# ai-decentralized/BloomBee

Measured on AMD Instinct MI355X. Metric: decode tokens/sec, llama-3-8b greedy, pipeline over RCCL/xGMI, higher is better.
Workload: dtype bfloat16; 1 GPU; model=llama-3-8b, global_batch=32, seq_len=2048, parallelism=pp1, micro_batches=1

## Files before the change

bloombee_amd/ops/hip/elementwise.hip:

```cpp

#include "common.h"


template <int BLOCK, int ITERS>
__global__ __launch_bounds__(BLOCK) void rmsnorm_kernel(
    const unsigned short* __restrict__ x, const unsigned short* __restrict__ res,
    const unsigned short* __restrict__ w, unsigned short* __restrict__ out_h,
    unsigned short* __restrict__ out_y, int H, float eps) {
  const long row = blockIdx.x;
  const unsigned short* xr = x + row * (long)H;
  const unsigned short* rr = res ? res + row * (long)H : nullptr;

  float v[ITERS][8];
  float ssq = 0.f;
#pragma unroll
  for (int it = 0; it < ITERS; ++it) {
    int d = (it * BLOCK + threadIdx.x) * 8;
    if (d < H) {
      load_bf16x8(xr + d, v[it]);
      if (rr) {
        float r[8];
        load_bf16x8(rr + d, r);
#pragma unroll
        for (int j = 0; j < 8; ++j) v[it][j] = bf2f(f2bf(v[it][j] + r[j]));
// ... 138 lines not shown
    for (int j = 0; j < 8; ++j) {
      float t = tanhf(0.7978845608028654f * (v[j] + 0.044715f * v[j] * v[j] * v[j]));
      o[j] = 0.5f * v[j] * (1.f + t);
    }
    store_bf16x8(out + idx * 8, o);
  }
  for (long i = nvec * 8 + blockIdx.x * (long)blockDim.x + threadIdx.x; i < n;
       i += (long)gridDim.x * blockDim.x) {
    const float v = bf2f(x[i]);
    const float t = tanhf(0.7978845608028654f * (v + 0.044715f * v * v * v));
    out[i] = f2bf(0.5f * v * (1.f + t));
  }
}

__global__ void add_kernel(const unsigned short* __restrict__ a,
                           const unsigned short* __restrict__ b,
                           unsigned short* __restrict__ out, long n) {
  const long nvec = n / 8;
  for (long idx = blockIdx.x * (long)blockDim.x + threadIdx.x; idx < nvec;
       idx += (long)gridDim.x * blockDim.x) {
    float va[8], vb[8], o[8];
    load_bf16x8(a + idx * 8, va);
    load_bf16x8(b + idx * 8, vb);
#pragma unroll
    for (int j = 0; j < 8; ++j) o[j] = va[j] + vb[j];
    store_bf16x8(out + idx * 8, o);
  }
  for (long i = nvec * 8 + blockIdx.x * (long)blockDim.x + threadIdx.x; i < n;
       i += (long)gridDim.x * blockDim.x)
    out[i] = f2bf(bf2f(a[i]) + bf2f(b[i]));
}


template <bool PART>
__global__ void rope_kv_write_kernel(
    unsigned short* __restrict__ qkv, const float* __restrict__ part,
    const unsigned short* __restrict__ bias, int ksplit,
    const float* __restrict__ cos_t,
    const float* __restrict__ sin_t, const int* __restrict__ pos,
    unsigned short* __restrict__ k_pages, unsigned short* __restrict__ v_pages,
    const int* __restrict__ page_table, const int* __restrict__ start_pos,
    int B, int Hq, int Hkv, int T, int D, int P, int maxp, int max_pos,
    int* __restrict__ ctx_out = nullptr) {
  constexpr int V = PART ? 4 : 1;
  const int bt = blockIdx.x;
  const int b = bt / T, t = bt % T;
  const int h = blockIdx.y;
  if (ctx_out && h == 0 && t == 0 && threadIdx.x == 0)
    ctx_out[b] = start_pos[b] + T;
  const int X = Hq + 2 * Hkv;
  const long hoff = (((long)b * T + t) * X + h) * D;
  unsigned short* base = qkv + hoff;
  auto load = [&](int i, float* x) {
    if constexpr (PART) {
      const long total = (long)B * T * X * D;
      f32x4 v = {0.f, 0.f, 0.f, 0.f};
      for (int s = 0; s < ksplit; ++s) {
        const f32x4 p =
            *reinterpret_cast<const f32x4*>(part + s * total + hoff + i);
#pragma unroll
        for (int e = 0; e < 4; ++e) v[e] += p[e];
      }
#pragma unroll
      for (int e = 0; e < 4; ++e) {
        if (bias) v[e] += bf2f(bias[h * D + i + e]);
        x[e] = bf2f(f2bf(v[e]));
      }
    } else {
      x[0] = bf2f(base[i]);
    }
  };

  const int abspos = start_pos[b] + t;
  if (h >= Hq + Hkv) {
    const int hv = h - Hq - Hkv;
    const int page = page_table[b * maxp + abspos / P];
    const int slot = abspos % P;
    unsigned short* dst = v_pages + ((long)page * Hkv + hv) * D * P + slot;
    for (int i = threadIdx.x * V; i < D; i += blockDim.x * V) {
      if constexpr (PART) {
        float x[V];
        load(i, x);
#pragma unroll
        for (int e = 0; e < V; ++e) dst[(long)(i + e) * P] = f2bf(x[e]);
      } else {
        dst[(long)i * P] = base[i];
      }
    }
    return;
  }
  const int p = min(max(pos ? pos[b * T + t] : abspos, 0), max_pos - 1);
  const float* c = cos_t + (long)p * (D / 2);
  const float* s = sin_t + (long)p * (D / 2);
  unsigned short* dst = base;
  if (h >= Hq) {
    const int hk = h - Hq;
    const int page = page_table[b * maxp + abspos / P];
    dst = k_pages + (((long)page * Hkv + hk) * P + (abspos % P)) * D;
  }
  for (int i = threadIdx.x * V; i < D / 2; i += blockDim.x * V) {
    float xa[V], xb[V];
    load(i, xa);
    load(i + D / 2, xb);
    unsigned short oa[V], ob[V];
#pragma unroll
    for (int e = 0; e < V; ++e) {
#pragma clang fp contract(off)
      float x1 = xa[e], x2 = xb[e];
      float cc = c[i + e], ss = s[i + e];
      oa[e] = f2bf(x1 * cc - x2 * ss);
      ob[e] = f2bf(x2 * cc + x1 * ss);
    }
    if constexpr (PART) {
      *reinterpret_cast<short4v*>(dst + i) =
          (short4v){(short)oa[0], (short)oa[1], (short)oa[2], (short)oa[3]};
      *reinterpret_cast<short4v*>(dst + i + D / 2) =
          (short4v){(short)ob[0], (short)ob[1], (short)ob[2], (short)ob[3]};
    } else {
      dst[i] = oa[0];
      dst[i + D / 2] = ob[0];
    }
  }
}
```

bloombee_amd/ops/hip/ext.hip:

```cpp

#include <torch/extension.h>
#include <c10/hip/HIPStream.h>
#include <hip/hip_runtime.h>
#include <cstdlib>

#include "common.h"

#include "elementwise.hip"
#include "kvcache.hip"
#include "attn_decode.hip"
#include "attn_decode_mfma.hip"
#include "attn_sparse.hip"
#include "attn_prefill.hip"
#include "attn_train.hip"
#include "gemm_skinny.hip"
#include "moe_gemm.hip"
#include "w4_gemm.hip"
#include "moe_gemm_w4.hip"
#include "mfma_selftest.hip"
#include "quant4.hip"
#include "wire.h"

typedef __attribute__((ext_vector_type(8))) short short8_h;

// ... 105 lines not shown

static SplitK split_k_chunks(int K, int unit, int ksplit) {
  const int nch = K / unit;
  TORCH_CHECK(nch >= 1 && ksplit >= 1, "split-K needs K >= ", unit);
  const int per = (nch + ksplit - 1) / ksplit;
  return {(nch + per - 1) / per, per * unit};
}

struct SkinnyPlan {
  int ksplit, kchunk;
  bool v2;
};

static SkinnyPlan skinny_plan(long N, long K, long ksplit_req) {
  TORCH_CHECK(N >= 64 && K >= 32 && K % 32 == 0 && N % 64 == 0,
              "K%32, N%64 required");
  int ksplit = (int)ksplit_req;
  if (ksplit <= 0) {
    static const int ks_big = [] {
      const char* e = std::getenv("BBAMD_GEMM_KSPLIT_BIG");
      return e ? std::atoi(e) : 1;
    }();
    if (N / 64 >= 256) ksplit = ks_big;
    else ksplit = (int)std::min<long>(K / 512,
                                      std::max<long>(1, std::min<long>(8, 1024 / (N / 64))));
    ksplit = std::max(1, ksplit);
  }
  if (K % 256 != 0)
    return {ksplit, (int)((K / 32 + ksplit - 1) / ksplit) * 32, false};
  const SplitK s = split_k_chunks((int)K, 256, ksplit);
  return {s.ksplit, s.kchunk, true};
}

struct W4Plan {
  bool gemv;
  int ksplit, kchunk;
};

static W4Plan w4_plan(long M, long N, long K, long ksplit_req) {
  TORCH_CHECK(N >= 64 && K >= 128 && K % 128 == 0 && N % 64 == 0,
              "K%128, N%64 required");
  if (M == 1 && K % 2048 == 0 && K / 2048 <= 7) return {true, 1, (int)K};
  int ksplit = (int)ksplit_req;
  if (ksplit <= 0) {
    ksplit = (int)std::max<long>(1, std::min<long>(K / 512, 1792 / (N / 64)));
  }
  const SplitK s = split_k_chunks((int)K, 128, ksplit);
  return {false, s.ksplit, s.kchunk};
}

static SplitK moe_w4_plan(long E, long N, long K, long S, long ksplit_req) {
  TORCH_CHECK(N >= 64 && K >= 128 && K % 128 == 0 && N % 64 == 0,
              "K%128, N%64 required");
  int ksplit = (int)ksplit_req;
  if (ksplit <= 0) {
    const long blocks = (N / 64) * std::max<long>(1, std::min<long>(E, S));
    ksplit = (int)std::max<long>(1, std::min<long>(K / 512, 1792 / blocks));
  }
  return split_k_chunks((int)K, 128, ksplit);
}

std::tuple<long, long, bool> gemm_skinny_plan(long N, long K, long ksplit_req) {
  const SkinnyPlan p = skinny_plan(N, K, ksplit_req);
  return {p.ksplit, p.kchunk, p.v2};
}

std::tuple<bool, long, long> gemm_w4_plan(long M, long N, long K, long ksplit_req) {
  const W4Plan p = w4_plan(M, N, K, ksplit_req);
  return {p.gemv, p.ksplit, p.kchunk};
}

std::tuple<long, long> moe_gemm_w4_plan(long E, long N, long K, long S,
                                        long ksplit_req) {
  const SplitK p = moe_w4_plan(E, N, K, S, ksplit_req);
  return {p.ksplit, p.kchunk};
}

struct Slabs {
  torch::Tensor t;
  float* p = nullptr;
};

static Slabs alloc_slabs(const Operands& ops, const torch::Tensor& like,
                         int ksplit, long rows, long N) {
  Slabs s;
  if (ksplit > 1) {
    s.t = torch::empty({(long)ksplit, rows, N}, like.options().dtype(at::kFloat));
    s.p = ops.ptr<F32>(s.t, "part");
  }
  return s;
}

static dim3 moe_grid(int N, long E, long mchunks, int ksplit) {
  TORCH_CHECK(mchunks >= 1 && E * mchunks <= 65535,
              "E * mchunks exceeds the grid limit");
  return dim3(N / 64, (unsigned)(E * mchunks), ksplit);
}
// ... 566 lines not shown
  auto* dvp = ops.ptr<Bf16>(dv, "dv");
  float* deltap = ops.ptr<F32>(delta, "delta");
  const int ntile = t.ntile;
  const int G = (int)(Hq / Hkv);
  dispatch_head_dim<128, 64>((int)D, "attn_train", [&](auto d) {
    constexpr int DD = decltype(d)::value;
    attn_train_dq_kernel<DD><<<(unsigned)(B * Hq * ntile), 512, 0, cur_stream()>>>(
        doutp, t.q, t.k, t.v, outp, lsep, alibi_ptr, dqp, deltap, (int)Hq, G,
        (int)T, ntile, (int)window, (float)scale,
        dout.stride(0), dout.stride(1), dout.stride(2),
        q.stride(0), q.stride(1), q.stride(2), k.stride(0), k.stride(1),
        k.stride(2), v.stride(0), v.stride(1), v.stride(2));
    attn_train_dkdv_kernel<DD><<<(unsigned)(B * Hkv * ntile), 512, 0, cur_stream()>>>(
        doutp, t.q, t.k, t.v, lsep, deltap, alibi_ptr, dkp, dvp,
        (int)Hq, G, (int)T, ntile, (int)window, (float)scale,
        dout.stride(0), dout.stride(1), dout.stride(2),
        q.stride(0), q.stride(1), q.stride(2), k.stride(0), k.stride(1),
        k.stride(2), v.stride(0), v.stride(1), v.stride(2));
  });
  return {dq, dk, dv};
}

static void rope_kv_write_launch(
    const Operands& ops, torch::Tensor& qkv, const float* partp, int nslab,
    const unsigned short* biasp, int* ctxp, int B, int T, int Hq, int Hkv,
    const torch::Tensor& cos_t, const torch::Tensor& sin_t,
    const c10::optional<torch::Tensor>& pos, const PagedKV& kv,
    const torch::Tensor& start_pos, long start_numel) {
  auto* qkvp = ops.ptr<Bf16>(qkv, "qkv");
  const float* cp = ops.ptr<F32>(cos_t, "cos_t");
  const float* sp = ops.ptr<F32>(sin_t, "sin_t");
  const int* posp = ops.ptr<I32>(pos, "pos", true, partp ? (long)B * T : -1);
  const int* spp = ops.ptr<I32>(start_pos, "start_pos", true, start_numel);
  dim3 grid(B * T, Hq + 2 * Hkv);
  if (partp)
    rope_kv_write_kernel<true><<<grid, 64, 0, cur_stream()>>>(
        qkvp, partp, biasp, nslab, cp, sp, posp, kv.k, kv.v, kv.pt, spp, B, Hq,
        Hkv, T, kv.D, kv.P, kv.maxp, (int)cos_t.size(0), ctxp);
  else
    rope_kv_write_kernel<false><<<grid, 64, 0, cur_stream()>>>(
        qkvp, nullptr, nullptr, 0, cp, sp, posp, kv.k, kv.v, kv.pt, spp, B, Hq,
        Hkv, T, kv.D, kv.P, kv.maxp, (int)cos_t.size(0));
}

void rope_kv_write_(torch::Tensor qkv, long Hq_, long Hkv_, torch::Tensor cos_t,
                    torch::Tensor sin_t, c10::optional<torch::Tensor> pos,
                    torch::Tensor k_pages, torch::Tensor v_pages,
                    torch::Tensor page_table, torch::Tensor start_pos) {
  Operands ops(qkv, "qkv");
  const PagedKV kv = paged_kv(ops, k_pages, v_pages, page_table);
  const int Hq = (int)Hq_, Hkv = (int)Hkv_;
  const int B = qkv.size(0), T = qkv.size(1);
  TORCH_CHECK(qkv.size(2) == (long)(Hq + 2 * Hkv) * kv.D, "bad fused qkv shape");
  rope_kv_write_launch(ops, qkv, nullptr, 0, nullptr, nullptr, B, T, Hq, Hkv,
                       cos_t, sin_t, pos, kv, start_pos, -1);
}

std::vector<torch::Tensor> rope_kv_write_part(torch::Tensor part,
                                 c10::optional<torch::Tensor> bias, long B_,
                                 long T_, long Hq_, long Hkv_,
                                 torch::Tensor cos_t, torch::Tensor sin_t,
                                 c10::optional<torch::Tensor> pos,
                                 torch::Tensor k_pages, torch::Tensor v_pages,
                                 torch::Tensor page_table,
                                 torch::Tensor start_pos) {
  Operands ops(part, "part");
  const float* partp = ops.ptr<F32>(part, "part");
  const PagedKV kv = paged_kv(ops, k_pages, v_pages, page_table);
  const int Hq = (int)Hq_, Hkv = (int)Hkv_, B = (int)B_, T = (int)T_;
  const int D = kv.D;
  const long X = Hq + 2 * Hkv;
  TORCH_CHECK(part.dim() == 3 && part.size(1) == (long)B * T &&
              part.size(2) == X * D,
              "part must be f32 (ksplit, B*T, (Hq+2Hkv)*D)");
  TORCH_CHECK(D % 8 == 0, "rope_kv_write_part needs head_dim % 8 == 0");
// ... 122 lines not shown
  dim3 grid(N / 64, ksplit);
  dispatch_mtile(M, [&](auto mt) {
    gemm_skinny_w4_kernel<decltype(mt)::value><<<grid, 256, 0, cur_stream()>>>(
        ap, qp, scp, zp, ksplit == 1 ? rp : nullptr, ksplit == 1 ? bp : nullptr,
        cp, part.p, M, N, K, plan.kchunk, ksplit);
  });
  if (ksplit > 1) {
    const long total = (long)M * N;
    const int cgrid = (int)std::min<long>((total + 255) / 256, 2048);
    gemm_skinny_combine_kernel<<<cgrid, 256, 0, cur_stream()>>>(
        part.p, rp, bp, cp, M, N, ksplit);
  }
  return C;
}


static const float* ss_in_operand(const Operands& ops,
                                  const c10::optional<torch::Tensor>& ss_in,
                                  int* nstripes) {
  *nstripes = 0;
  if (!ss_in.has_value()) return nullptr;
  TORCH_CHECK(ss_in->numel() % 32 == 0, "ss_in must be f32 (nstripes,32)");
  *nstripes = (int)(ss_in->numel() / 32);
  return ops.ptr<F32>(*ss_in, "ss_in");
}

torch::Tensor gemm_skinny(torch::Tensor A, torch::Tensor W,
                          c10::optional<torch::Tensor> residual,
                          c10::optional<torch::Tensor> bias, long ksplit_req,
                          c10::optional<torch::Tensor> norm_w, double eps,
                          c10::optional<torch::Tensor> ss_in,
                          c10::optional<torch::Tensor> ss_out,
                          long norm_mode_req, bool defer_combine,
                          c10::optional<torch::Tensor> cnt) {
  Operands ops(A, "A");
  const auto* ap = ops.ptr<Bf16>(A, "A");
  const auto* wp = ops.ptr<Bf16>(W, "W");
  const int K = A.size(-1);
  const int M = A.numel() / K;
  const int N = W.size(0);
  TORCH_CHECK(M <= 32, "gemm_skinny is for M <= 32, got ", M);
  TORCH_CHECK(W.size(1) == K, "A/W K mismatch");
  TORCH_CHECK(K % 32 == 0 && N % 64 == 0, "K%32, N%64 required");
  int norm_mode = (int)norm_mode_req;
  const auto* nwp = ops.ptr<Bf16>(norm_w, "norm_w", true, K);
  if (nwp && norm_mode == 0) norm_mode = 1;
  TORCH_CHECK(norm_mode != 1 || nwp, "norm_mode 1 needs norm_w");
  if (norm_mode)
    TORCH_CHECK(K % 256 == 0, "fused rmsnorm needs the v2 (K%256) kernel");
  TORCH_CHECK(!ss_in.has_value() || norm_mode != 0,
              "ss_in only meaningful with a norm mode");
  int nstripes = 0;
  const float* ssinp = ss_in_operand(ops, ss_in, &nstripes);
  float* ssoutp = ops.ptr<F32>(ss_out, "ss_out", true, (long)(N / 64) * 32);
  const auto* rp = ops.ptr<Bf16>(residual, "residual", true, (long)M * N);
  const auto* bp = ops.ptr<Bf16>(bias, "bias", true, N);
  int* cntp = ops.ptr<I32>(cnt, "cnt");
  auto sizes = A.sizes().vec();
  sizes.back() = N;
  auto C = torch::empty(sizes, A.options());
  auto* cp = ops.ptr<Bf16>(C, "C");
  const SkinnyPlan plan = skinny_plan(N, K, ksplit_req);
  const int ksplit = plan.ksplit, kchunk = plan.kchunk;
  const Slabs part = alloc_slabs(ops, A, ksplit, M, N);
  if (cnt.has_value() && ksplit > 1 && plan.v2) {
    TORCH_CHECK(!defer_combine, "cnt and defer_combine exclude each other");
    TORCH_CHECK(cnt->numel() >= N / 64, "cnt must be int32 of >= N/64 entries");
    dispatch_mtile(M, [&](auto mt) {
      gemm_skinny_v2_kernel<decltype(mt)::value, 2>
          <<<dim3((N / 64) * ksplit), 256, 0, cur_stream()>>>(
              ap, wp, rp, bp, cp, part.p, M, N, K, kchunk, ksplit, nwp,
              (float)eps, norm_mode, ssinp, nstripes, ssoutp, cntp);
    });
    return C;
  }
  dim3 grid(N / 64, ksplit);
  dispatch_mtile(M, [&](auto mt) {
    if (plan.v2)
      gemm_skinny_v2_kernel<decltype(mt)::value><<<grid, 256, 0, cur_stream()>>>(
          ap, wp, ksplit == 1 ? rp : nullptr, ksplit == 1 ? bp : nullptr, cp,
          part.p, M, N, K, kchunk, ksplit, nwp, (float)eps, norm_mode, ssinp,
          nstripes, ksplit == 1 ? ssoutp : nullptr);
    else {
      TORCH_CHECK(!norm_mode && (!ssoutp || ksplit > 1),
                  "fused norm / ss_out need the v2 (K%256) kernel");
      gemm_skinny_kernel<decltype(mt)::value><<<grid, 256, 0, cur_stream()>>>(
          ap, wp, ksplit == 1 ? rp : nullptr, ksplit == 1 ? bp : nullptr, cp,
          part.p, M, N, K, ksplit);
    }
  });
  if (ksplit > 1 && defer_combine) {
    TORCH_CHECK(!rp && !ssoutp, "defer_combine takes no residual / ss_out");
    return part.t;
  }
  if (ksplit > 1) {
    if (ssoutp || (N % 64 == 0 && N / 64 >= 64)) {
      dim3 cg(N / 64, (M + 15) / 16);
      gemm_skinny_combine_ss_kernel<<<cg, 256, 0, cur_stream()>>>(
          part.p, rp, bp, cp, ssoutp, M, N, ksplit);
    } else {
      const long total = (long)M * N;
      const int cgrid = (int)std::min<long>((total + 255) / 256, 2048);
      gemm_skinny_combine_kernel<<<cgrid, 256, 0, cur_stream()>>>(
          part.p, rp, bp, cp, M, N, ksplit);
    }
  }
  return C;
}

torch::Tensor gemm_skinny_swiglu(torch::Tensor A, torch::Tensor W, double eps,
                                 c10::optional<torch::Tensor> ss_in,
                                 long norm_mode_req) {
  Operands ops(A, "A");
  const auto* ap = ops.ptr<Bf16>(A, "A");
  const auto* wp = ops.ptr<Bf16>(W, "W");
  const int K = A.size(-1);
  const int M = A.numel() / K;
  const int N = W.size(0);
  const int I = N / 2;
  const int norm_mode = (int)norm_mode_req;
  TORCH_CHECK(M >= 1 && M <= 32, "gemm_skinny_swiglu is for 1 <= M <= 32, got ", M);
  TORCH_CHECK(W.dim() == 2 && W.size(1) == K, "A/W K mismatch");
  TORCH_CHECK(N % 2 == 0 && I % 32 == 0 && K % 256 == 0,
              "gemm_skinny_swiglu needs I % 32 == 0 and K % 256 == 0");
  TORCH_CHECK(norm_mode == 0 || norm_mode == 2, "norm_mode must be 0 or 2");
  TORCH_CHECK(!ss_in.has_value() || norm_mode == 2,
              "ss_in only meaningful with norm_mode 2");
  int nstripes = 0;
  const float* ssinp = ss_in_operand(ops, ss_in, &nstripes);
  auto sizes = A.sizes().vec();
  sizes.back() = I;
  auto C = torch::empty(sizes, A.options());
  auto* cp = ops.ptr<Bf16>(C, "C");
  dispatch_mtile(M, [&](auto mt) {
    gemm_skinny_v2_kernel<decltype(mt)::value, 1>
        <<<dim3(I / 32), 256, 0, cur_stream()>>>(
            ap, wp, nullptr, nullptr, cp, nullptr, M, N, K, K, 1, nullptr,
            (float)eps, norm_mode, ssinp, nstripes, nullptr, nullptr);
  });
  return C;
}


std::vector<torch::Tensor> quant4_pack(torch::Tensor x) {
  Operands ops(x, "x");
  const auto* xp = ops.ptr<Bf16>(x, "x");
  const long ncols = x.size(-1);
  TORCH_CHECK(ncols % 64 == 0, "quant4 needs cols % 64 == 0");
  const long nrows = x.numel() / ncols;
  auto packed = torch::empty({nrows, ncols / 2}, x.options().dtype(at::kByte));
  auto scale = torch::empty({nrows, ncols / 64}, x.options().dtype(at::kHalf));
  auto zero = torch::empty_like(scale);
  const long ngroups = nrows * (ncols / 64);
  const int wpb = 4;
  quant4_pack_kernel<64><<<(ngroups + wpb - 1) / wpb, wpb * 64, 0, cur_stream()>>>(
      xp, ops.ptr<U8>(packed, "packed"), ops.ptr<F16>(scale, "scale"),
      ops.ptr<F16>(zero, "zero"), nrows, ncols);
  return {packed, scale, zero};
}

torch::Tensor quant4_unpack(torch::Tensor packed, torch::Tensor scale,
                            torch::Tensor zero) {
  Operands ops(packed, "packed");
  auto* qp = ops.ptr<U8>(packed, "packed");
  TORCH_CHECK(packed.dim() == 2, "packed must be (rows, cols/2)");
  const long nrows = packed.size(0), ncols = packed.size(1) * 2;
  TORCH_CHECK(ncols % 64 == 0, "quant4 needs cols % 64 == 0");
  auto* scp = ops.ptr<F16>(scale, "scale", true, nrows * (ncols / 64));
  auto* zp = ops.ptr<F16>(zero, "zero", true, nrows * (ncols / 64));
  auto out = torch::empty({nrows, ncols}, packed.options().dtype(at::kBFloat16));
  const long total = nrows * ncols;
// ... 32 lines not shown
  mfma_selftest_kernel<<<1, 64, 0, cur_stream()>>>(ap, bp, ops.ptr<F32>(C, "C"));
  return C;
}

PYBIND11_MODULE(TORCH_EXTENSION_NAME, m) {
  m.def("rms_norm", &rms_norm);
  m.def("rms_norm_residual", &rms_norm_residual);
  m.def("layer_norm", &layer_norm);
  m.def("rope_apply_", &rope_apply_);
  m.def("swiglu", &swiglu);
  m.def("gelu_tanh", &gelu_tanh);
  m.def("add_bf16", &add_bf16);
  m.def("kv_write", &kv_write);
  m.def("kv_gather", &kv_gather);
  m.def("wire_deflate", &wire_deflate);
  m.def("wire_inflate", &wire_inflate);
  m.def("wire_deflate_mt", &wire_deflate_mt);
  m.def("wire_inflate_mt", &wire_inflate_mt);
  m.def("attn_decode", &attn_decode);
  m.def("attn_decode_qkv", &attn_decode_qkv);
  m.def("attn_decode_mixed", &attn_decode_mixed);
  m.def("attn_decode_sparse", &attn_decode_sparse);
  m.def("attn_decode_sparse_qkv", &attn_decode_sparse_qkv);
  m.def("attn_prefill_qkv", &attn_prefill_qkv);
  m.def("rope_kv_write_", &rope_kv_write_);
  m.def("attn_prefill", &attn_prefill);
  m.def("attn_train_fwd", &attn_train_fwd);
  m.def("attn_train_bwd", &attn_train_bwd);
  m.def("gemm_skinny", &gemm_skinny, py::arg("A"), py::arg("W"),
        py::arg("residual") = c10::nullopt, py::arg("bias") = c10::nullopt,
        py::arg("ksplit") = 0, py::arg("norm_w") = c10::nullopt,
        py::arg("eps") = 0.0, py::arg("ss_in") = c10::nullopt,
        py::arg("ss_out") = c10::nullopt, py::arg("norm_mode") = 0,
        py::arg("defer_combine") = false, py::arg("cnt") = c10::nullopt);
  m.def("gemm_skinny_swiglu", &gemm_skinny_swiglu, py::arg("A"), py::arg("W"),
        py::arg("eps") = 0.0, py::arg("ss_in") = c10::nullopt,
        py::arg("norm_mode") = 0);
  m.def("gemm_skinny_plan", &gemm_skinny_plan);
  m.def("rope_kv_write_part", &rope_kv_write_part);
  m.def("moe_gemm", &moe_gemm);
  m.def("gemm_w4", &gemm_w4);
  m.def("gemm_w4_plan", &gemm_w4_plan);
  m.def("moe_gemm_w4", &moe_gemm_w4);
  m.def("moe_gemm_w4_plan", &moe_gemm_w4_plan);
  m.def("quant4_pack", &quant4_pack);
  m.def("quant4_unpack", &quant4_unpack);
  m.def("mfma_selftest", &mfma_selftest);
  m.def("kv_stream_probe", &kv_stream_probe);
}
```

bloombee_amd/ops/hip/gemm_skinny.hip:

```cpp

#include "common.h"

template <int MT>
__global__ __launch_bounds__(256) void gemm_skinny_kernel(
    const unsigned short* __restrict__ A,
    const unsigned short* __restrict__ W,
    const unsigned short* __restrict__ R,
    const unsigned short* __restrict__ bias,
    unsigned short* __restrict__ C,
    float* __restrict__ Cpart,
    int M, int N, int K, int ksplit) {
  const int wave = threadIdx.x / WAVE;
  const int lane = threadIdx.x & (WAVE - 1);
  const int li = lane & 15;
  const int hi = lane >> 4;
  const int n0 = blockIdx.x * 64 + wave * 16;
  if (n0 >= N) return;
  const int split = blockIdx.y;
  const int kchunk = ((K / 32 + ksplit - 1) / ksplit) * 32;
  const int k0 = split * kchunk;
  const int k1 = min(K, k0 + kchunk);

  const unsigned short* wrow = W + (long)(n0 + li) * K;
  int arow[MT];
// ... 58 lines not shown

DEVINL void gemm_skinny_combine_lane(
    const float* Cpart, const unsigned short* __restrict__ R,
    const unsigned short* __restrict__ bias, unsigned short* __restrict__ C,
    float* __restrict__ ssout, int M, int N, int ksplit, int stripe, int m,
    int lane) {
  const int n0 = stripe * 64;
  const int c4 = (lane & 15) * 4;
  const long total = (long)M * N;
  const long i = (long)m * N + n0 + c4;
  f32x4 v = {0.f, 0.f, 0.f, 0.f};
  for (int s = 0; s < ksplit; ++s) {
    const f32x4 p = *reinterpret_cast<const f32x4*>(Cpart + s * total + i);
#pragma unroll
    for (int e = 0; e < 4; ++e) v[e] += p[e];
  }
#pragma unroll
  for (int e = 0; e < 4; ++e) {
    if (bias) v[e] += bf2f(bias[n0 + c4 + e]);
    if (R) v[e] += bf2f(R[i + e]);
  }
  short4v o4;
#pragma unroll
  for (int e = 0; e < 4; ++e) o4[e] = (short)f2bf(v[e]);
  *reinterpret_cast<short4v*>(C + i) = o4;
  if (ssout) {
    float vs = v[0] * v[0] + v[1] * v[1] + v[2] * v[2] + v[3] * v[3];
#pragma unroll
    for (int msk = 1; msk < 16; msk <<= 1) vs += __shfl_xor(vs, msk);
    if ((lane & 15) == 0) ssout[(long)stripe * 32 + m] = vs;
  }
}

template <int MT, int EPI = 0>
__global__ __launch_bounds__(256) void gemm_skinny_v2_kernel(
    const unsigned short* __restrict__ A,
    const unsigned short* __restrict__ W,
    const unsigned short* __restrict__ R,
    const unsigned short* __restrict__ bias,
    unsigned short* __restrict__ C,
    float* __restrict__ Cpart,
    int M, int N, int K, int kchunk, int ksplit,
    const unsigned short* __restrict__ nw,
    float eps, int norm_mode,
    const float* __restrict__ ssin,
    int nstripes,
    float* __restrict__ ssout,
    int* cnt = nullptr) {
  constexpr int U = 4;
  constexpr int KSTEP = 256;
  constexpr int RSTRIDE = KSTEP + 8;
  __shared__ __attribute__((aligned(16))) unsigned short atile[32 * RSTRIDE];
  __shared__ float ssp[256];
  __shared__ float invr[32];

  const int wave = threadIdx.x / WAVE;
  const int lane = threadIdx.x & (WAVE - 1);
  const int li = lane & 15;
  const int hi = lane >> 4;
  int tile = blockIdx.x;
  {
    const int nwg = gridDim.x;
    const int xcd = tile % 8, orig8 = tile / 8;
    const int q = nwg / 8, r = nwg % 8;
    if (nwg >= 8)
      tile = (xcd < r ? xcd * (q + 1) : r * (q + 1) + (xcd - r) * q) + orig8;
  }
  int split = blockIdx.y;
  if constexpr (EPI == 2) {
    split = tile % ksplit;
    tile /= ksplit;
  }
  const int n0 = tile * 64 + wave * 16;
  const int k0 = split * kchunk;
  const int k1 = min(K, k0 + kchunk);

  const unsigned short* wrow = W + (long)(n0 + li) * K;
  if constexpr (EPI == 1)
    wrow = W + ((long)(li < 8 ? 0 : N / 2 - 8) + tile * 32 + wave * 8 + li) * K;

  f32x4 acc[MT];
#pragma unroll
  for (int t = 0; t < MT; ++t) acc[t] = (f32x4){0.f, 0.f, 0.f, 0.f};

  short8 aregs[(32 * KSTEP) / (256 * 8)];
  short8 nregs[(32 * KSTEP) / (256 * 8)];
  auto load_a = [&](int ks) {
#pragma unroll
    for (int j = 0; j < 4; ++j) {
      const int flat = threadIdx.x + j * 256;
      const int row = min(flat / 32, M - 1);
      const int off = (flat % 32) * 8;
      aregs[j] = *reinterpret_cast<const short8*>(A + (long)row * K + ks + off);
      if (norm_mode == 1)
        nregs[j] = *reinterpret_cast<const short8*>(nw + ks + off);
    }
  };
  auto store_a = [&]() {
#pragma unroll
    for (int j = 0; j < 4; ++j) {
      const int flat = threadIdx.x + j * 256;
      short8 v = aregs[j];
      if (norm_mode == 1) {
        const float ir = invr[flat / 32 >= M ? M - 1 : flat / 32];
#pragma unroll
        for (int e = 0; e < 8; ++e)
          v[e] = (short)f2bf(bf2f((unsigned short)v[e]) * ir *
                             bf2f((unsigned short)nregs[j][e]));
      }
      *reinterpret_cast<short8*>(atile + (flat / 32) * RSTRIDE + (flat % 32) * 8) =
          v;
    }
  };

  bf16x8 bB0[U], bB1[U];
  auto issue0 = [&](int k) {
#pragma unroll
    for (int u = 0; u < U; ++u)
      bB0[u] = as_bf16x8(
          *reinterpret_cast<const short8*>(wrow + k + u * 32 + hi * 8));
  };
  auto issue1 = [&](int k) {
#pragma unroll
    for (int u = 0; u < U; ++u)
      bB1[u] = as_bf16x8(
          *reinterpret_cast<const short8*>(wrow + k + u * 32 + hi * 8));
  };
  auto mfma_set = [&](bf16x8* bB, int half) {
#pragma unroll
    for (int u = 0; u < U; ++u)
#pragma unroll
      for (int t = 0; t < MT; ++t) {
        bf16x8 afrag = as_bf16x8(*reinterpret_cast<const short8*>(
            atile + (t * 16 + li) * RSTRIDE + half * 128 + u * 32 + hi * 8));
        acc[t] = __builtin_amdgcn_mfma_f32_16x16x32_bf16(afrag, bB[u], acc[t],
                                                         0, 0, 0);
      }
  };

  auto reduce_invr = [&]() {
    if (ssin) {
      const int row = threadIdx.x & 31, grp = threadIdx.x >> 5;
      float s0 = 0.f, s1 = 0.f, s2 = 0.f, s3 = 0.f;
      int s = grp;
// ... 9 lines not shown
      if (threadIdx.x < 32) {
        float t = 0.f;
#pragma unroll
        for (int g = 0; g < 8; ++g) t += ssp[g * 32 + threadIdx.x];
        invr[threadIdx.x] = rsqrtf(t / K + eps);
      }
      __syncthreads();
    } else {
      const int row = threadIdx.x >> 3, sub = threadIdx.x & 7;
      float ss = 0.f;
      if (row < M) {
        const unsigned short* p = A + (long)row * K + sub * (K / 8);
        for (int x = 0; x < K / 8; x += 8) {
          short8 v = *reinterpret_cast<const short8*>(p + x);
#pragma unroll
          for (int e = 0; e < 8; ++e) {
            const float f = bf2f((unsigned short)v[e]);
            ss += f * f;
          }
        }
      }
      ssp[threadIdx.x] = ss;
      __syncthreads();
      if (sub == 0 && row < M) {
        float t = 0.f;
#pragma unroll
        for (int e = 0; e < 8; ++e) t += ssp[(row << 3) + e];
        invr[row] = rsqrtf(t / K + eps);
      }
      __syncthreads();
    }
  };

  if (norm_mode == 1) {
    issue0(k0);
    reduce_invr();
    load_a(k0);
    store_a();
    __syncthreads();
  } else {
    load_a(k0);
    issue0(k0);
    store_a();
    __syncthreads();
  }
  for (int k = k0; k < k1; k += KSTEP) {
    if (k + KSTEP < k1) load_a(k + KSTEP);
    issue1(k + 128);
    mfma_set(bB0, 0);
    if (k + KSTEP < k1) issue0(k + KSTEP);
    mfma_set(bB1, 1);
    if (k + KSTEP < k1) {
      __syncthreads();
      store_a();
      __syncthreads();
    }
  }

  if (norm_mode == 2) reduce_invr();

  if constexpr (EPI == 1) {
    unsigned short* otile = atile;
    __syncthreads();
#pragma unroll
    for (int t = 0; t < MT; ++t)
#pragma unroll
      for (int reg = 0; reg < 4; ++reg) {
        const int m = t * 16 + hi * 4 + reg;
        float v = acc[t][reg];
        if (norm_mode == 2) v *= invr[m];
        const float g = bf2f(f2bf(v));
        const float u = __shfl_xor(g, 8);
        const float sg = g / (1.f + fast_expf(-g));
        if (li < 8) otile[m * 32 + wave * 8 + li] = f2bf(sg * u);
      }
    __syncthreads();
    if (threadIdx.x < 128) {
      const int m = threadIdx.x >> 2, c8 = (threadIdx.x & 3) * 8;
      if (m < M)
        *reinterpret_cast<short8*>(C + (long)m * (N / 2) + tile * 32 + c8) =
            *reinterpret_cast<const short8*>(otile + m * 32 + c8);
    }
    return;
  }

  if constexpr (EPI == 2) {
    constexpr int TS = 68;
    float* ftile = reinterpret_cast<float*>(atile);
    __syncthreads();
// ... 69 lines not shown
          if (m < M) {
            float v = acc[t][reg];
            if (norm_mode == 2) v *= invr[m];
            if (bias) v += bf2f(bias[n0 + li]);
            if (R) v += bf2f(R[(long)m * N + n0 + li]);
            C[(long)m * N + n0 + li] = f2bf(v);
            vs = v * v;
          }
#pragma unroll
          for (int msk = 1; msk < 16; msk <<= 1) vs += __shfl_xor(vs, msk);
          if (li == 0) ssp[wave * 32 + m] = vs;
        }
      __syncthreads();
      if (threadIdx.x < 32)
        ssout[(long)tile * 32 + threadIdx.x] =
            ssp[threadIdx.x] + ssp[32 + threadIdx.x] +
            ssp[64 + threadIdx.x] + ssp[96 + threadIdx.x];
    }
  } else {
    float* dst = Cpart + (long)split * M * N;
#pragma unroll
    for (int t = 0; t < MT; ++t)
#pragma unroll
      for (int reg = 0; reg < 4; ++reg) {
        const int m = t * 16 + hi * 4 + reg;
        if (m >= M) continue;
        float v = acc[t][reg];
        if (norm_mode == 2) v *= invr[m];
        dst[(long)m * N + n0 + li] = v;
      }
  }
}

__global__ __launch_bounds__(256) void gemm_skinny_combine_ss_kernel(
    const float* __restrict__ Cpart, const unsigned short* __restrict__ R,
    const unsigned short* __restrict__ bias, unsigned short* __restrict__ C,
    float* __restrict__ ssout, int M, int N, int ksplit) {
  const int lane = threadIdx.x & (WAVE - 1);
  const int m = blockIdx.y * 16 + (threadIdx.x >> 6) * 4 + (lane >> 4);
  if (m >= M) return;
  gemm_skinny_combine_lane(Cpart, R, bias, C, ssout, M, N, ksplit, blockIdx.x,
                           m, lane);
}

__global__ void gemm_skinny_combine_kernel(
    const float* __restrict__ Cpart, const unsigned short* __restrict__ R,
    const unsigned short* __restrict__ bias, unsigned short* __restrict__ C,
    int M, int N, int ksplit) {
  const long total = (long)M * N;
  for (long i = blockIdx.x * (long)blockDim.x + threadIdx.x; i < total;
       i += (long)gridDim.x * blockDim.x) {
    float v = 0.f;
    for (int s = 0; s < ksplit; ++s) v += Cpart[(long)s * total + i];
    if (bias) v += bf2f(bias[i % N]);
    if (R) v += bf2f(R[i]);
    C[i] = f2bf(v);
  }
}
```

Measured before the change: 5417 tokens/s.

## Add configurable W-ring prefetch depth to skinny GEMM and vectorize split-K rope write

```diff
diff --git a/bloombee_amd/ops/hip/elementwise.hip b/bloombee_amd/ops/hip/elementwise.hip
--- a/bloombee_amd/ops/hip/elementwise.hip
+++ b/bloombee_amd/ops/hip/elementwise.hip
@@ -194,44 +194,18 @@
 }
 
 
-template <bool PART>
 __global__ void rope_kv_write_kernel(
-    unsigned short* __restrict__ qkv, const float* __restrict__ part,
-    const unsigned short* __restrict__ bias, int ksplit,
-    const float* __restrict__ cos_t,
+    unsigned short* __restrict__ qkv, const float* __restrict__ cos_t,
     const float* __restrict__ sin_t, const int* __restrict__ pos,
     unsigned short* __restrict__ k_pages, unsigned short* __restrict__ v_pages,
     const int* __restrict__ page_table, const int* __restrict__ start_pos,
-    int B, int Hq, int Hkv, int T, int D, int P, int maxp, int max_pos,
-    int* __restrict__ ctx_out = nullptr) {
-  constexpr int V = PART ? 4 : 1;
+    int B, int Hq, int Hkv, int T, int D, int P, int maxp, int max_pos) {
   const int bt = blockIdx.x;
   const int b = bt / T, t = bt % T;
   const int h = blockIdx.y;
-  if (ctx_out && h == 0 && t == 0 && threadIdx.x == 0)
-    ctx_out[b] = start_pos[b] + T;
   const int X = Hq + 2 * Hkv;
   const long hoff = (((long)b * T + t) * X + h) * D;
   unsigned short* base = qkv + hoff;
-  auto load = [&](int i, float* x) {
-    if constexpr (PART) {
-      const long total = (long)B * T * X * D;
-      f32x4 v = {0.f, 0.f, 0.f, 0.f};
-      for (int s = 0; s < ksplit; ++s) {
-        const f32x4 p =
-            *reinterpret_cast<const f32x4*>(part + s * total + hoff + i);
-#pragma unroll
-        for (int e = 0; e < 4; ++e) v[e] += p[e];
-      }
-#pragma unroll
-      for (int e = 0; e < 4; ++e) {
-        if (bias) v[e] += bf2f(bias[h * D + i + e]);
-        x[e] = bf2f(f2bf(v[e]));
-      }
-    } else {
-      x[0] = bf2f(base[i]);
-    }
-  };
 
   const int abspos = start_pos[b] + t;
   if (h >= Hq + Hkv) {
@@ -239,16 +213,7 @@
     const int page = page_table[b * maxp + abspos / P];
     const int slot = abspos % P;
     unsigned short* dst = v_pages + ((long)page * Hkv + hv) * D * P + slot;
-    for (int i = threadIdx.x * V; i < D; i += blockDim.x * V) {
-      if constexpr (PART) {
-        float x[V];
-        load(i, x);
-#pragma unroll
-        for (int e = 0; e < V; ++e) dst[(long)(i + e) * P] = f2bf(x[e]);
-      } else {
-        dst[(long)i * P] = base[i];
-      }
-    }
+    for (int i = threadIdx.x; i < D; i += blockDim.x) dst[(long)i * P] = base[i];
     return;
   }
   const int p = min(max(pos ? pos[b * T + t] : abspos, 0), max_pos - 1);
@@ -260,27 +225,103 @@
     const int page = page_table[b * maxp + abspos / P];
     dst = k_pages + (((long)page * Hkv + hk) * P + (abspos % P)) * D;
   }
-  for (int i = threadIdx.x * V; i < D / 2; i += blockDim.x * V) {
-    float xa[V], xb[V];
-    load(i, xa);
-    load(i + D / 2, xb);
-    unsigned short oa[V], ob[V];
-#pragma unroll
-    for (int e = 0; e < V; ++e) {
+  for (int i = threadIdx.x; i < D / 2; i += blockDim.x) {
 #pragma clang fp contract(off)
-      float x1 = xa[e], x2 = xb[e];
-      float cc = c[i + e], ss = s[i + e];
-      oa[e] = f2bf(x1 * cc - x2 * ss);
-      ob[e] = f2bf(x2 * cc + x1 * ss);
-    }
-    if constexpr (PART) {
-      *reinterpret_cast<short4v*>(dst + i) =
-          (short4v){(short)oa[0], (short)oa[1], (short)oa[2], (short)oa[3]};
-      *reinterpret_cast<short4v*>(dst + i + D / 2) =
-          (short4v){(short)ob[0], (short)ob[1], (short)ob[2], (short)ob[3]};
-    } else {
-      dst[i] = oa[0];
-      dst[i + D / 2] = ob[0];
-    }
-  }
-}
+    float x1 = bf2f(base[i]), x2 = bf2f(base[i + D / 2]);
+    float cc = c[i], ss = s[i];
+    dst[i] = f2bf(x1 * cc - x2 * ss);
+    dst[i + D / 2] = f2bf(x2 * cc + x1 * ss);
+  }
+}
+
+__global__ __launch_bounds__(256) void rope_kv_write_part_kernel(
+    unsigned short* __restrict__ qkv, const float* __restrict__ part,
+    const unsigned short* __restrict__ bias, int ksplit,
+    const float* __restrict__ cos_t, const float* __restrict__ sin_t,
+    const int* __restrict__ pos, unsigned short* __restrict__ k_pages,
+    unsigned short* __restrict__ v_pages, const int* __restrict__ page_table,
+    const int* __restrict__ start_pos, int B, int Hq, int Hkv, int T, int D,
+    int P, int maxp, int max_pos, int* __restrict__ ctx_out) {
+  constexpr int NS = 8;
+  const int bt = blockIdx.x;
+  const int b = bt / T, t = bt % T;
+  if (blockIdx.y == 0 && t == 0 && threadIdx.x == 0)
+    ctx_out[b] = start_pos[b] + T;
+  const int X = Hq + 2 * Hkv;
+  const int item = blockIdx.y * blockDim.x + threadIdx.x;
+  if (item >= X * (D / 8)) return;
+  const int h = item / (D / 8);
+  const int i = (item % (D / 8)) * 4;
+  const long total = (long)B * T * X * D;
+  const long hoff = ((long)bt * X + h) * D;
+
+  f32x4 pa[NS], pb[NS];
+#pragma unroll
+  for (int s = 0; s < NS; ++s) {
+    const float* src = part + min(s, ksplit - 1) * total + hoff + i;
+    pa[s] = *reinterpret_cast<const f32x4*>(src);
+    pb[s] = *reinterpret_cast<const f32x4*>(src + D / 2);
+  }
+  f32x4 va = {0.f, 0.f, 0.f, 0.f}, vb = {0.f, 0.f, 0.f, 0.f};
+#pragma unroll
+  for (int s = 0; s < NS; ++s)
+    if (s < ksplit) {
+#pragma unroll
+      for (int e = 0; e < 4; ++e) {
+        va[e] += pa[s][e];
+        vb[e] += pb[s][e];
+      }
+    }
+  for (int s = NS; s < ksplit; ++s) {
+    const float* src = part + s * total + hoff + i;
+    const f32x4 qa = *reinterpret_cast<const f32x4*>(src);
+    const f32x4 qb = *reinterpret_cast<const f32x4*>(src + D / 2);
+#pragma unroll
+    for (int e = 0; e < 4; ++e) {
+      va[e] += qa[e];
+      vb[e] += qb[e];
+    }
+  }
+  unsigned short ra[4], rb[4];
+#pragma unroll
+  for (int e = 0; e < 4; ++e) {
+    if (bias) {
+      va[e] += bf2f(bias[h * D + i + e]);
+      vb[e] += bf2f(bias[h * D + i + D / 2 + e]);
+    }
+    ra[e] = f2bf(va[e]);
+    rb[e] = f2bf(vb[e]);
+  }
+
+  const int abspos = start_pos[b] + t;
+  if (h >= Hq + Hkv) {
+    const int hv = h - Hq - Hkv;
+    const int page = page_table[b * maxp + abspos / P];
+    unsigned short* dst = v_pages + ((long)page * Hkv + hv) * D * P + abspos % P;
+#pragma unroll
+    for (int e = 0; e < 4; ++e) {
+      dst[(long)(i + e) * P] = ra[e];
+      dst[(long)(i + D / 2 + e) * P] = rb[e];
+    }
+    return;
+  }
+  const int p = min(max(pos ? pos[b * T + t] : abspos, 0), max_pos - 1);
+  const float* c = cos_t + (long)p * (D / 2);
+  const float* s = sin_t + (long)p * (D / 2);
+  unsigned short* dst = qkv + hoff;
+  if (h >= Hq) {
+    const int page = page_table[b * maxp + abspos / P];
+    dst = k_pages + (((long)page * Hkv + (h - Hq)) * P + (abspos % P)) * D;
+  }
+  short4v oa, ob;
+#pragma unroll
+  for (int e = 0; e < 4; ++e) {
+#pragma clang fp contract(off)
+    float x1 = bf2f(ra[e]), x2 = bf2f(rb[e]);
+    float cc = c[i + e], ss = s[i + e];
+    oa[e] = (short)f2bf(x1 * cc - x2 * ss);
+    ob[e] = (short)f2bf(x2 * cc + x1 * ss);
+  }
+  *reinterpret_cast<short4v*>(dst + i) = oa;
+  *reinterpret_cast<short4v*>(dst + i + D / 2) = ob;
+}
diff --git a/bloombee_amd/ops/hip/ext.hip b/bloombee_amd/ops/hip/ext.hip
--- a/bloombee_amd/ops/hip/ext.hip
+++ b/bloombee_amd/ops/hip/ext.hip
@@ -161,6 +161,29 @@
   return {s.ksplit, s.kchunk, true};
 }
 
+static constexpr int kWringDepths[] = {2, 4};
+
+static int skinny_wring(long req) {
+  static const int env = [] {
+    const char* e = std::getenv("BBAMD_GEMM_WRING");
+    return e ? std::atoi(e) : 0;
+  }();
+  if (req <= 0) req = env;
+  if (req <= 0) return 2;
+  TORCH_CHECK(std::find(std::begin(kWringDepths), std::end(kWringDepths), req) !=
+                  std::end(kWringDepths),
+              "gemm_skinny W ring depth must be 2 or 4, got ", req);
+  return (int)req;
+}
+
+template <int MT, int EPI, typename... Args>
+static void launch_skinny_v2(int depth, dim3 grid, Args... args) {
+  if (depth == 2)
+    gemm_skinny_v2_kernel<MT, EPI><<<grid, 256, 0, cur_stream()>>>(args...);
+  else
+    gemm_skinny_v2_ring_kernel<MT, EPI, 4><<<grid, 256, 0, cur_stream()>>>(args...);
+}
+
 struct W4Plan {
   bool gemv;
   int ksplit, kchunk;
@@ -192,6 +215,15 @@
 std::tuple<long, long, bool> gemm_skinny_plan(long N, long K, long ksplit_req) {
   const SkinnyPlan p = skinny_plan(N, K, ksplit_req);
   return {p.ksplit, p.kchunk, p.v2};
+}
+
+std::tuple<long, std::vector<long>> gemm_skinny_wring_plan(long N, long K,
+                                                           long ksplit_req,
+                                                           long wring_req) {
+  const SkinnyPlan p = skinny_plan(N, K, ksplit_req);
+  const std::vector<long> built(std::begin(kWringDepths), std::end(kWringDepths));
+  if (!p.v2) return {0, built};
+  return {skinny_wring(wring_req), built};
 }
 
 std::tuple<bool, long, long> gemm_w4_plan(long M, long N, long K, long ksplit_req) {
@@ -824,15 +856,18 @@
   const float* sp = ops.ptr<F32>(sin_t, "sin_t");
   const int* posp = ops.ptr<I32>(pos, "pos", true, partp ? (long)B * T : -1);
   const int* spp = ops.ptr<I32>(start_pos, "start_pos", true, start_numel);
-  dim3 grid(B * T, Hq + 2 * Hkv);
-  if (partp)
-    rope_kv_write_kernel<true><<<grid, 64, 0, cur_stream()>>>(
+  if (partp) {
+    const int items = (Hq + 2 * Hkv) * (kv.D / 8);
+    dim3 grid(B * T, (items + 255) / 256);
+    rope_kv_write_part_kernel<<<grid, 256, 0, cur_stream()>>>(
         qkvp, partp, biasp, nslab, cp, sp, posp, kv.k, kv.v, kv.pt, spp, B, Hq,
         Hkv, T, kv.D, kv.P, kv.maxp, (int)cos_t.size(0), ctxp);
-  else
-    rope_kv_write_kernel<false><<<grid, 64, 0, cur_stream()>>>(
-        qkvp, nullptr, nullptr, 0, cp, sp, posp, kv.k, kv.v, kv.pt, spp, B, Hq,
-        Hkv, T, kv.D, kv.P, kv.maxp, (int)cos_t.size(0));
+  } else {
+    dim3 grid(B * T, Hq + 2 * Hkv);
+    rope_kv_write_kernel<<<grid, 64, 0, cur_stream()>>>(
+        qkvp, cp, sp, posp, kv.k, kv.v, kv.pt, spp, B, Hq, Hkv, T, kv.D, kv.P,
+        kv.maxp, (int)cos_t.size(0));
+  }
 }
 
 void rope_kv_write_(torch::Tensor qkv, long Hq_, long Hkv_, torch::Tensor cos_t,
@@ -1021,7 +1056,7 @@
                           c10::optional<torch::Tensor> ss_in,
                           c10::optional<torch::Tensor> ss_out,
                           long norm_mode_req, bool defer_combine,
-                          c10::optional<torch::Tensor> cnt) {
+                          c10::optional<torch::Tensor> cnt, long wring_req) {
   Operands ops(A, "A");
   const auto* ap = ops.ptr<Bf16>(A, "A");
   const auto* wp = ops.ptr<Bf16>(W, "W");
@@ -1052,24 +1087,30 @@
   const SkinnyPlan plan = skinny_plan(N, K, ksplit_req);
   const int ksplit = plan.ksplit, kchunk = plan.kchunk;
   const Slabs part = alloc_slabs(ops, A, ksplit, M, N);
+  const int wring =
+      !plan.v2 ? 0
+      : norm_mode == 1
+          ? 2
+          : skinny_wring(wring_req);
   if (cnt.has_value() && ksplit > 1 && plan.v2) {
     TORCH_CHECK(!defer_combine, "cnt and defer_combine exclude each other");
     TORCH_CHECK(cnt->numel() >= N / 64, "cnt must be int32 of >= N/64 entries");
     dispatch_mtile(M, [&](auto mt) {
-      gemm_skinny_v2_kernel<decltype(mt)::value, 2>
-          <<<dim3((N / 64) * ksplit), 256, 0, cur_stream()>>>(
-              ap, wp, rp, bp, cp, part.p, M, N, K, kchunk, ksplit, nwp,
-              (float)eps, norm_mode, ssinp, nstripes, ssoutp, cntp);
+      launch_skinny_v2<decltype(mt)::value, 2>(
+          wring, dim3((N / 64) * ksplit), ap, wp, rp, bp, cp, part.p, M, N, K,
+          kchunk, ksplit, nwp, (float)eps, norm_mode, ssinp, nstripes, ssoutp,
+          cntp);
     });
     return C;
   }
   dim3 grid(N / 64, ksplit);
   dispatch_mtile(M, [&](auto mt) {
     if (plan.v2)
-      gemm_skinny_v2_kernel<decltype(mt)::value><<<grid, 256, 0, cur_stream()>>>(
-          ap, wp, ksplit == 1 ? rp : nullptr, ksplit == 1 ? bp : nullptr, cp,
-          part.p, M, N, K, kchunk, ksplit, nwp, (float)eps, norm_mode, ssinp,
-          nstripes, ksplit == 1 ? ssoutp : nullptr);
+      launch_skinny_v2<decltype(mt)::value, 0>(
+          wring, grid, ap, wp, ksplit == 1 ? rp : nullptr,
+          ksplit == 1 ? bp : nullptr, cp, part.p, M, N, K, kchunk, ksplit, nwp,
+          (float)eps, norm_mode, ssinp, nstripes,
+          ksplit == 1 ? ssoutp : nullptr, (int*)nullptr);
     else {
       TORCH_CHECK(!norm_mode && (!ssoutp || ksplit > 1),
                   "fused norm / ss_out need the v2 (K%256) kernel");
@@ -1099,7 +1140,7 @@
 
 torch::Tensor gemm_skinny_swiglu(torch::Tensor A, torch::Tensor W, double eps,
                                  c10::optional<torch::Tensor> ss_in,
-                                 long norm_mode_req) {
+                                 long norm_mode_req, long wring_req) {
   Operands ops(A, "A");
   const auto* ap = ops.ptr<Bf16>(A, "A");
   const auto* wp = ops.ptr<Bf16>(W, "W");
@@ -1121,11 +1162,13 @@
   sizes.back() = I;
   auto C = torch::empty(sizes, A.options());
   auto* cp = ops.ptr<Bf16>(C, "C");
+  const int wring = skinny_wring(wring_req);
   dispatch_mtile(M, [&](auto mt) {
-    gemm_skinny_v2_kernel<decltype(mt)::value, 1>
-        <<<dim3(I / 32), 256, 0, cur_stream()>>>(
-            ap, wp, nullptr, nullptr, cp, nullptr, M, N, K, K, 1, nullptr,
-            (float)eps, norm_mode, ssinp, nstripes, nullptr, nullptr);
+    launch_skinny_v2<decltype(mt)::value, 1>(
+        wring, dim3(I / 32), ap, wp, (const unsigned short*)nullptr,
+        (const unsigned short*)nullptr, cp, (float*)nullptr, M, N, K, K, 1,
+        (const unsigned short*)nullptr, (float)eps, norm_mode, ssinp, nstripes,
+        (float*)nullptr, (int*)nullptr);
   });
   return C;
 }
@@ -1224,11 +1267,14 @@
         py::arg("ksplit") = 0, py::arg("norm_w") = c10::nullopt,
         py::arg("eps") = 0.0, py::arg("ss_in") = c10::nullopt,
         py::arg("ss_out") = c10::nullopt, py::arg("norm_mode") = 0,
-        py::arg("defer_combine") = false, py::arg("cnt") = c10::nullopt);
+        py::arg("defer_combine") = false, py::arg("cnt") = c10::nullopt,
+        py::arg("wring") = 0);
   m.def("gemm_skinny_swiglu", &gemm_skinny_swiglu, py::arg("A"), py::arg("W"),
         py::arg("eps") = 0.0, py::arg("ss_in") = c10::nullopt,
-        py::arg("norm_mode") = 0);
+        py::arg("norm_mode") = 0, py::arg("wring") = 0);
   m.def("gemm_skinny_plan", &gemm_skinny_plan);
+  m.def("gemm_skinny_wring_plan", &gemm_skinny_wring_plan, py::arg("N"),
+        py::arg("K"), py::arg("ksplit") = 0, py::arg("wring") = 0);
   m.def("rope_kv_write_part", &rope_kv_write_part);
   m.def("moe_gemm", &moe_gemm);
   m.def("gemm_w4", &gemm_w4);
diff --git a/bloombee_amd/ops/hip/gemm_skinny.hip b/bloombee_amd/ops/hip/gemm_skinny.hip
--- a/bloombee_amd/ops/hip/gemm_skinny.hip
+++ b/bloombee_amd/ops/hip/gemm_skinny.hip
@@ -114,8 +114,21 @@
   }
 }
 
-template <int MT, int EPI = 0>
-__global__ __launch_bounds__(256) void gemm_skinny_v2_kernel(
+template <int I>
+struct WringIdx {
+  static constexpr int value = I;
+};
+
+template <int DEPTH, int N, typename F>
+DEVINL void wring_tail_dispatch(int nrem, F& f) {
+  if constexpr (N <= 2 * DEPTH - 2) {
+    if (nrem == N) f(WringIdx<N>{});
+    else wring_tail_dispatch<DEPTH, N + 2>(nrem, f);
+  }
+}
+
+template <int MT, int EPI, int DEPTH>
+DEVINL void gemm_skinny_v2_body(
     const unsigned short* __restrict__ A,
     const unsigned short* __restrict__ W,
     const unsigned short* __restrict__ R,
@@ -128,10 +141,13 @@
     const float* __restrict__ ssin,
     int nstripes,
     float* __restrict__ ssout,
-    int* cnt = nullptr) {
+    int* cnt) {
+  static_assert(DEPTH == 2 || DEPTH % 4 == 0, "ring: whole waves per A row");
   constexpr int U = 4;
-  constexpr int KSTEP = 256;
+  constexpr int KSTEP = DEPTH * 128;
   constexpr int RSTRIDE = KSTEP + 8;
+  constexpr int RPIECE = KSTEP / 8;
+  constexpr int NPIECE = (32 * KSTEP) / (256 * 8);
   __shared__ __attribute__((aligned(16))) unsigned short atile[32 * RSTRIDE];
   __shared__ float ssp[256];
   __shared__ float invr[32];
@@ -165,33 +181,43 @@
 #pragma unroll
   for (int t = 0; t < MT; ++t) acc[t] = (f32x4){0.f, 0.f, 0.f, 0.f};
 
-  short8 aregs[(32 * KSTEP) / (256 * 8)];
-  short8 nregs[(32 * KSTEP) / (256 * 8)];
-  auto load_a = [&](int ks) {
-#pragma unroll
-    for (int j = 0; j < 4; ++j) {
-      const int flat = threadIdx.x + j * 256;
-      const int row = min(flat / 32, M - 1);
-      const int off = (flat % 32) * 8;
-      aregs[j] = *reinterpret_cast<const short8*>(A + (long)row * K + ks + off);
-      if (norm_mode == 1)
-        nregs[j] = *reinterpret_cast<const short8*>(nw + ks + off);
+  short8 aregs[NPIECE];
+  short8 nregs[DEPTH == 2 ? NPIECE : 1];
+  const int wave_s = __builtin_amdgcn_readfirstlane(wave);
+  auto load_a = [&](int ks, int lim = 1 << 30) {
+#pragma unroll
+    for (int j = 0; j < NPIECE; ++j) {
+      if constexpr (DEPTH == 2) {
+        const int flat = threadIdx.x + j * 256;
+        const int row = min(flat / RPIECE, M - 1);
+        const int off = (flat % RPIECE) * 8;
+        aregs[j] = *reinterpret_cast<const short8*>(A + (long)row * K + ks + off);
+        if (norm_mode == 1)
+          nregs[j] = *reinterpret_cast<const short8*>(nw + ks + off);
+      } else {
+        const int fw = wave_s + j * 4;
+        const int row = min(fw / (RPIECE / 64), M - 1);
+        const unsigned off =
+            min((fw % (RPIECE / 64)) * 64 + lane, lim / 8 - 1) * 16u;
+        aregs[j] = *reinterpret_cast<const short8*>(
+            reinterpret_cast<const char*>(A + (long)row * K + ks) + off);
+      }
     }
   };
   auto store_a = [&]() {
 #pragma unroll
-    for (int j = 0; j < 4; ++j) {
+    for (int j = 0; j < NPIECE; ++j) {
       const int flat = threadIdx.x + j * 256;
       short8 v = aregs[j];
-      if (norm_mode == 1) {
-        const float ir = invr[flat / 32 >= M ? M - 1 : flat / 32];
+      if (DEPTH == 2 && norm_mode == 1) {
+        const float ir = invr[flat / RPIECE >= M ? M - 1 : flat / RPIECE];
 #pragma unroll
         for (int e = 0; e < 8; ++e)
           v[e] = (short)f2bf(bf2f((unsigned short)v[e]) * ir *
                              bf2f((unsigned short)nregs[j][e]));
       }
-      *reinterpret_cast<short8*>(atile + (flat / 32) * RSTRIDE + (flat % 32) * 8) =
-          v;
+      *reinterpret_cast<short8*>(atile + (flat / RPIECE) * RSTRIDE +
+                                 (flat % RPIECE) * 8) = v;
     }
   };
 
@@ -267,29 +293,88 @@
     }
   };
 
-  if (norm_mode == 1) {
-    issue0(k0);
-    reduce_invr();
-    load_a(k0);
+  if constexpr (DEPTH == 2) {
+    if (norm_mode == 1) {
+      issue0(k0);
+      reduce_invr();
+      load_a(k0);
+      store_a();
+      __syncthreads();
+    } else {
+      load_a(k0);
+      issue0(k0);
+      store_a();
+      __syncthreads();
+    }
+    for (int k = k0; k < k1; k += KSTEP) {
+      if (k + KSTEP < k1) load_a(k + KSTEP);
+      issue1(k + 128);
+      mfma_set(bB0, 0);
+      if (k + KSTEP < k1) issue0(k + KSTEP);
+      mfma_set(bB1, 1);
+      if (k + KSTEP < k1) {
+        __syncthreads();
+        store_a();
+        __syncthreads();
+      }
+    }
+  } else {
+    bf16x8 ring[DEPTH][U];
+    auto issue = [&](int j, int k) {
+#pragma unroll
+      for (int u = 0; u < U; ++u)
+        ring[j][u] = as_bf16x8(
+            *reinterpret_cast<const short8*>(wrow + k + u * 32 + hi * 8));
+    };
+    auto issue_ring = [&]() {
+#pragma unroll
+      for (int j = 0; j < DEPTH; ++j) issue(j, min(k0 + j * 128, k1 - 128));
+      __builtin_amdgcn_sched_barrier(0);
+    };
+    load_a(k0, min(KSTEP, k1 - k0));
+    __builtin_amdgcn_sched_barrier(0);
+    issue_ring();
     store_a();
     __syncthreads();
-  } else {
-    load_a(k0);
-    issue0(k0);
-    store_a();
-    __syncthreads();
-  }
-  for (int k = k0; k < k1; k += KSTEP) {
-    if (k + KSTEP < k1) load_a(k + KSTEP);
-    issue1(k + 128);
-    mfma_set(bB0, 0);
-    if (k + KSTEP < k1) issue0(k + KSTEP);
-    mfma_set(bB1, 1);
-    if (k + KSTEP < k1) {
+    int k = k0;
+    for (; k + 2 * KSTEP <= k1; k += KSTEP) {
+      load_a(k + KSTEP);
+      __builtin_amdgcn_sched_barrier(0);
+#pragma unroll
+      for (int j = 0; j < DEPTH; ++j) {
+        mfma_set(ring[j], j);
+        issue(j, k + KSTEP + j * 128);
+        __builtin_amdgcn_sched_barrier(0);
+      }
       __syncthreads();
       store_a();
       __syncthreads();
     }
+    auto tail = [&](auto nrem_c) {
+      constexpr int NREM = decltype(nrem_c)::value;
+      constexpr int CUR = NREM < DEPTH ? NREM : DEPTH;
+      constexpr int NEXT = NREM - CUR;
+      if constexpr (NEXT > 0) {
+        load_a(k + KSTEP, NEXT * 128);
+        __builtin_amdgcn_sched_barrier(0);
+      }
+#pragma unroll
+      for (int j = 0; j < CUR; ++j) {
+        mfma_set(ring[j], j);
+        if (j < NEXT) {
+          issue(j, k + KSTEP + j * 128);
+          __builtin_amdgcn_sched_barrier(0);
+        }
+      }
+      if constexpr (NEXT > 0) {
+        __syncthreads();
+        store_a();
+        __syncthreads();
+#pragma unroll
+        for (int j = 0; j < NEXT; ++j) mfma_set(ring[j], j);
+      }
+    };
+    wring_tail_dispatch<DEPTH, 2>((k1 - k) / 128, tail);
   }
 
   if (norm_mode == 2) reduce_invr();
@@ -425,6 +510,29 @@
   }
 }
 
+#define SKINNY_V2_PARAMS                                                      \
+  const unsigned short *__restrict__ A, const unsigned short *__restrict__ W, \
+      const unsigned short *__restrict__ R,                                   \
+      const unsigned short *__restrict__ bias, unsigned short *__restrict__ C, \
+      float *__restrict__ Cpart, int M, int N, int K, int kchunk, int ksplit, \
+      const unsigned short *__restrict__ nw, float eps, int norm_mode,        \
+      const float *__restrict__ ssin, int nstripes, float *__restrict__ ssout, \
+      int *cnt
+#define SKINNY_V2_ARGS                                                       \
+  A, W, R, bias, C, Cpart, M, N, K, kchunk, ksplit, nw, eps, norm_mode, ssin, \
+      nstripes, ssout, cnt
+
+template <int MT, int EPI = 0>
+__global__ __launch_bounds__(256) void gemm_skinny_v2_kernel(SKINNY_V2_PARAMS) {
+  gemm_skinny_v2_body<MT, EPI, 2>(SKINNY_V2_ARGS);
+}
+
+template <int MT, int EPI, int DEPTH>
+__global__ __launch_bounds__(256, 3) void gemm_skinny_v2_ring_kernel(
+    SKINNY_V2_PARAMS) {
+  gemm_skinny_v2_body<MT, EPI, DEPTH>(SKINNY_V2_ARGS);
+}
+
 __global__ __launch_bounds__(256) void gemm_skinny_combine_ss_kernel(
     const float* __restrict__ Cpart, const unsigned short* __restrict__ R,
     const unsigned short* __restrict__ bias, unsigned short* __restrict__ C,
```

Result: faster. 5477 tokens/s (median of 6 runs) (+1.1%).
